# facebookresearch/robust-dynrf

Hardware: AMD Instinct MI355X
Metric: training rays/sec (Nvidia Balloon1, configs/Nvidia.txt, static+dynamic TensorVMSplit) (higher is better)
Workload: dtype f32; 1 GPU; BASELINE.json configs[1]: Nvidia Balloon1, configs/Nvidia.txt, 4096 rays/iter/GPU, 1xMI355X per rank, static+dynamic TensorVMSplit; one step = 5 dynamic + 5 static forward passes, scene-flow MLP, induced flow/disparity, per-frame depth loss, distortion loss, compositor, factor regularisers, full backward, Adam; config=nvidia, stage=stage0, samples_per_ray=115, global_batch=4096, rays_per_gpu=4096, parallelism=ray-sharded dp1, ranks=1, dead_work=executed (work the reference also computes although nothing consumes it)

## Files before the change

include/rodynrf.h:

```cpp
#ifndef RODYNRF_H
#define RODYNRF_H
#include <stddef.h>
#include <stdint.h>

#ifdef __cplusplus
extern "C" {
#endif

#define RDRF_ABI_VERSION 6

typedef void* rdrf_stream_t;

enum { RDRF_RAY_NDC = 0, RDRF_RAY_CONTRACT = 1, RDRF_RAY_OTHER = 2 };
enum { RDRF_ACT_RELU = 0, RDRF_ACT_SOFTPLUS = 1 };
enum { RDRF_HEAD_MLP_FEA = 0, RDRF_HEAD_MLP_FEA_TIMEEMBEDDING = 1 };
enum { RDRF_SCATTER_RAY = 0, RDRF_SCATTER_SORTED = 1, RDRF_SCATTER_AUTO = 2, RDRF_SCATTER_SORTED_PLAIN = 3 };

typedef struct {
  float* plane[3];
  float* line[3];
  int C[3];
  int H[3], W[3];
  int L[3];
  int sH[3], sW[3];
// ... 307 lines not shown
  const uint8_t* masks;
} RdrfSceneTables;
typedef struct RdrfBatch {
  float* rgb;
  float* disp;
  float* fg;
  float* mask_f;
  float* mask_b;
  float* flow_f;
  float* flow_b;
  float* ts;
  float* ts_rand;
  float* grid;
  float* px;
  int64_t* view;
} RdrfBatch;
int rdrf_gather_batch(const RdrfSceneTables* tables, const int64_t* ids, const int64_t* ids2, int N, RdrfBatch* out,
                      rdrf_stream_t stream);

int rdrf_set_scatter_mode(int mode);

int rdrf_deterministic(void);
int rdrf_det_bind(int slot, float* grad_base, size_t n, void* shadow_i64, rdrf_stream_t stream);
int rdrf_det_finish(int slot, rdrf_stream_t stream);

int rdrf_selftest_mlp(const float* x, const float* w, const float* b, int M, int K, int OUT,
                      float* y, void* ws, size_t ws_bytes, rdrf_stream_t stream);

#define RDRF_ST_F32 0
#define RDRF_ST_F32_T 1
#define RDRF_ST_B3 2
#define RDRF_ST_B3_T 3
#define RDRF_ST_B3_PAIR_T 4
#define RDRF_ST_B3S 5
#define RDRF_ST_B3S_T 6
int rdrf_selftest_layer(int form, const float* x, const float* w, int M, int K, int OUT, float* y, void* ws, size_t ws_bytes,
                        rdrf_stream_t stream);

#define RDRF_DW_DENSITY 0
#define RDRF_DW_STATIC_FEA 1
#define RDRF_DW_STATIC_TE 2
#define RDRF_DW_DYN_APP 3
#define RDRF_DW_DYN 4
#define RDRF_DW_SCENE_FLOW 5
#define RDRF_DW_FEAT_STATIC 6
#define RDRF_DW_FEAT_DYN 7
#define RDRF_DW_LIVE_D 1
#define RDRF_DW_LIVE_B 2
#define RDRF_DW_SMALL_IN_KERNEL 4
#define RDRF_DW_WARP_IN_KERNEL 8
int rdrf_selftest_dw(int plan, int flags, const float* A, size_t A_floats, const float* B, size_t B_floats, int ntiles,
                     const int* count, const void* grads, rdrf_stream_t stream);
int rdrf_selftest_dw_describe(int plan, int flags, int* out, int cap);
int rdrf_selftest_sf_geometry(int ntiles, int* grid, int* waves);
int rdrf_selftest_warp_geometry(int ntiles, int* grid, int* waves);
size_t rdrf_selftest_warp_bwd_workspace_bytes(int N, int S);
int rdrf_selftest_warp_bwd(const RdrfDynamicParams* P, const RdrfFieldCfg* cfg, int N, int S, const float* act1,
                           size_t act1_floats, float* grows1, size_t grows1_floats, float* dxw, float* dxn,
                           const float* g_xyz_prime, const RdrfDynamicParams* grads, float* g_xyz, float* dtout, float* dtp,
                           void* ws, size_t ws_bytes, rdrf_stream_t stream);

size_t rdrf_selftest_sort_temp_bytes(unsigned n, int bits);
int rdrf_selftest_sort(const unsigned* keys, unsigned n, int bits, const int* count, unsigned n_mul, unsigned* keys_out,
                       unsigned* order, void* temp, size_t temp_bytes, rdrf_stream_t stream);

#define RDRF_SCK_STATIC_DENSITY 0
#define RDRF_SCK_DYN_DENSITY 1
#define RDRF_SCK_STATIC_APP 2
#define RDRF_SCK_DYN_APP 3
typedef struct {
  RdrfVM vm[2], gvm[2];
  int set_mask;
  int N, S, flat;
  const float* coords;
  float box_lo[3], box_inv[3];
  const unsigned char* valid;
  const int* list;
  const int* count;
  const float* rows;
  size_t rows_floats;
  const float* recs;
  size_t recs_floats;
  float* dxw;
  float* g_xyz;
  void* ws;
  size_t ws_bytes;
  unsigned* keys_out;
  unsigned* keys_sorted_out;
  unsigned* order_out;
  int* counts_out;
} RdrfScatterTest;
size_t rdrf_selftest_scatter_workspace_bytes(int N, int S);
int rdrf_selftest_scatter(int kind, int mode, const RdrfScatterTest* t, rdrf_stream_t stream);
int rdrf_selftest_scatter_describe(int kind, const int* grid, int* out, int cap);
int rdrf_selftest_scatter_last(int* out, int cap);

typedef struct RdrfAlphaMask {
  const uint8_t* bits;
  int grid[3];
  int T;
  float aabb[6];
} RdrfAlphaMask;

size_t rdrf_compute_alpha_workspace_bytes(int M, int T);
int rdrf_compute_alpha(const void* params, int dynamic, const RdrfFieldCfg* cfg, const float* xyz, int M,
                       const float* times, int T, float length, const RdrfAlphaMask* mask, float* alpha, float* sigma,
// ... 19 lines not shown
```

robust-dynrf_amd/_lib.py:

```python
import ctypes as C
import os

import torch

_HERE = os.path.dirname(os.path.abspath(__file__))
DETERMINISTIC = os.environ.get("RDRF_DETERMINISTIC", "0") == "1"
LIB_PATH = os.environ.get("RDRF_LIB", os.path.join(_HERE, "librodynrf_det.so" if DETERMINISTIC else "librodynrf.so"))

ABI_VERSION = 6

RAY_TYPES = {"ndc": 0, "contract": 1}
ACTS = {"relu": 0, "softplus": 1}
HEADS = {"MLP_Fea": 0, "MLP_Fea_TimeEmbedding": 1}
SAVE_NO_APP = 1

fp = C.POINTER(C.c_float)


class RdrfVM(C.Structure):
    _fields_ = [("plane", C.c_void_p * 3), ("line", C.c_void_p * 3), ("C", C.c_int * 3),
                ("H", C.c_int * 3), ("W", C.c_int * 3), ("L", C.c_int * 3),
                ("sH", C.c_int * 3), ("sW", C.c_int * 3)]


# ... 98 lines not shown
                                   C.c_void_p]
    lib.rdrf_pack_floats.restype = C.c_size_t
    lib.rdrf_pack_floats.argtypes = []
    lib.rdrf_loss_terms_workspace_floats.restype = C.c_size_t
    lib.rdrf_loss_terms_workspace_floats.argtypes = [C.c_int]
    lib.rdrf_frame_depth_loss_workspace_bytes.restype = C.c_size_t
    lib.rdrf_frame_depth_loss_workspace_bytes.argtypes = [C.c_int, C.c_int]
    lib.rdrf_frame_depth_loss_fwd.argtypes = [C.c_void_p, C.c_void_p, C.c_void_p, C.c_void_p, C.c_int, C.c_int, C.c_float,
                                              C.c_void_p, C.c_void_p, C.c_void_p, C.c_size_t, C.c_void_p]
    lib.rdrf_frame_depth_loss_bwd.argtypes = [C.c_void_p, C.c_void_p, C.c_void_p, C.c_int, C.c_float, C.c_void_p, C.c_void_p]
    lib.rdrf_render_workspace_bytes.restype = C.c_size_t
    lib.rdrf_render_workspace_bytes.argtypes = [C.c_int, C.c_int]
    lib.rdrf_render_chunks_workspace_bytes.restype = C.c_size_t
    lib.rdrf_render_chunks_workspace_bytes.argtypes = [C.c_int, C.c_int, C.c_int]
    lib.rdrf_render_maps_fwd.argtypes = [C.c_void_p, C.c_void_p, C.c_void_p, C.c_void_p, C.c_void_p, C.c_void_p, C.c_int,
                                         C.c_int, C.c_float, C.c_float, C.c_int, C.POINTER(RenderMapsC), C.c_void_p,
                                         C.c_size_t, C.c_void_p]
    lib.rdrf_render_chunks_maps_fwd.argtypes = [C.c_void_p, C.c_void_p, C.c_void_p, C.c_void_p, C.c_void_p, C.c_void_p,
                                                C.c_int, C.c_int, C.c_int, C.c_float, C.c_float, C.POINTER(RenderMapsC),
                                                C.c_void_p, C.c_size_t, C.c_void_p, C.c_void_p, C.c_int]
    lib.rdrf_render_world_fwd.argtypes = [C.c_void_p, C.c_void_p, C.c_void_p, C.c_void_p, C.c_void_p, C.c_void_p, C.c_int,
                                          C.c_int, C.c_int, C.c_float, C.c_float, C.c_float, C.c_int, C.POINTER(RenderMapsC),
                                          C.c_void_p, C.c_size_t, C.c_void_p, C.c_void_p, C.c_int]
    lib.rdrf_render_motion_workspace_bytes.restype = C.c_size_t
    lib.rdrf_render_motion_workspace_bytes.argtypes = [C.c_int, C.c_int]
    lib.rdrf_render_motion_fwd.argtypes = [C.c_void_p, C.c_void_p, C.c_void_p, C.c_void_p, C.c_void_p, C.c_void_p, C.c_int,
                                           C.c_int, C.c_float, C.c_float, C.c_int, C.POINTER(RenderMapsC),
                                           C.POINTER(MotionCamsC), C.POINTER(MotionMapsC), C.c_void_p, C.c_size_t, C.c_void_p]
    lib.rdrf_flow_to_image_workspace_bytes.restype = C.c_size_t
    lib.rdrf_flow_to_image_workspace_bytes.argtypes = [C.c_int, C.c_int]
    lib.rdrf_flow_to_image.argtypes = [C.c_void_p, C.c_int, C.c_int, C.c_void_p, C.c_void_p, C.c_size_t, C.c_void_p]
    lib.rdrf_camera_rays.argtypes = [C.c_void_p, C.c_void_p, C.c_int, C.c_int, C.c_int, C.c_int, C.c_float, C.c_int64,
                                     C.c_int, C.c_void_p, C.c_void_p]
    lib.rdrf_ssim_workspace_bytes.restype = C.c_size_t
    lib.rdrf_ssim_workspace_bytes.argtypes = [C.c_int, C.c_int, C.c_int]
    lib.rdrf_ssim.argtypes = [C.c_void_p, C.c_void_p, C.c_int, C.c_int, C.c_int, C.c_float, C.c_void_p, C.c_void_p,
                              C.c_void_p, C.c_size_t, C.c_void_p]
    lib.rdrf_compute_alpha_workspace_bytes.restype = C.c_size_t
    lib.rdrf_compute_alpha_workspace_bytes.argtypes = [C.c_int, C.c_int]
    lib.rdrf_compute_alpha.argtypes = [C.c_void_p, C.c_int, C.c_void_p, C.c_void_p, C.c_int, C.c_void_p, C.c_int, C.c_float,
                                       C.POINTER(RdrfAlphaMask), C.c_void_p, C.c_void_p, C.c_void_p, C.c_size_t, C.c_void_p]
    lib.rdrf_alpha_mask_build.argtypes = [C.c_void_p, C.c_int, C.c_int, C.c_int, C.c_int, C.c_float, C.c_void_p, C.c_void_p,
                                          C.c_void_p]
    lib.rdrf_alpha_mask_sample.argtypes = [C.POINTER(RdrfAlphaMask), C.c_void_p, C.c_void_p, C.c_int, C.c_int64, C.c_void_p,
                                           C.c_void_p]
    lib.rdrf_alpha_mask_valid.argtypes = [C.POINTER(RdrfAlphaMask), C.POINTER(RdrfAlphaMask), C.c_void_p, C.c_void_p, C.c_int,
                                          C.c_int, C.c_void_p, C.c_void_p]
    lib.rdrf_gather_batch.argtypes = [C.POINTER(SceneTablesC), C.c_void_p, C.c_void_p, C.c_int, C.POINTER(BatchC), C.c_void_p]
    lib.rdrf_selftest_layer.argtypes = [C.c_int, C.c_void_p, C.c_void_p, C.c_int, C.c_int, C.c_int, C.c_void_p, C.c_void_p,
                                        C.c_size_t, C.c_void_p]
    lib.rdrf_selftest_dw.argtypes = [C.c_int, C.c_int, C.c_void_p, C.c_size_t, C.c_void_p, C.c_size_t, C.c_int, C.c_void_p,
                                     C.c_void_p, C.c_void_p]
    lib.rdrf_selftest_dw_describe.argtypes = [C.c_int, C.c_int, C.POINTER(C.c_int), C.c_int]
    lib.rdrf_selftest_warp_geometry.argtypes = [C.c_int, C.POINTER(C.c_int), C.POINTER(C.c_int)]
    lib.rdrf_selftest_warp_bwd_workspace_bytes.restype = C.c_size_t
    lib.rdrf_selftest_warp_bwd_workspace_bytes.argtypes = [C.c_int, C.c_int]
    lib.rdrf_selftest_warp_bwd.argtypes = [C.c_void_p, C.c_void_p, C.c_int, C.c_int, C.c_void_p, C.c_size_t, C.c_void_p, C.c_size_t,
                                           C.c_void_p, C.c_void_p, C.c_void_p, C.c_void_p, C.c_void_p, C.c_void_p, C.c_void_p,
                                           C.c_void_p, C.c_size_t, C.c_void_p]
    lib.rdrf_selftest_sort_temp_bytes.restype = C.c_size_t
    lib.rdrf_selftest_sort_temp_bytes.argtypes = [C.c_uint, C.c_int]
    lib.rdrf_selftest_sort.argtypes = [C.c_void_p, C.c_uint, C.c_int, C.c_void_p, C.c_uint, C.c_void_p, C.c_void_p, C.c_void_p,
                                       C.c_size_t, C.c_void_p]
    lib.rdrf_selftest_scatter_workspace_bytes.restype = C.c_size_t
    lib.rdrf_selftest_scatter_workspace_bytes.argtypes = [C.c_int, C.c_int]
    lib.rdrf_selftest_scatter.argtypes = [C.c_int, C.c_int, C.POINTER(RdrfScatterTest), C.c_void_p]
    lib.rdrf_selftest_scatter_describe.argtypes = [C.c_int, C.POINTER(C.c_int), C.POINTER(C.c_int), C.c_int]
    lib.rdrf_selftest_scatter_last.argtypes = [C.POINTER(C.c_int), C.c_int]
    lib.rdrf_prof_get.argtypes = [C.c_char_p, C.POINTER(C.c_double), C.POINTER(C.c_int)]
    lib.rdrf_det_bind.argtypes = [C.c_int, C.c_void_p, C.c_size_t, C.c_void_p, C.c_void_p]
    lib.rdrf_det_finish.argtypes = [C.c_int, C.c_void_p]
    if DETERMINISTIC and not lib.rdrf_deterministic():
        raise ImportError(f"RDRF_DETERMINISTIC=1 but {LIB_PATH} is the product build")
    return lib


lib = _load()

SYMBOLS = [
    "rdrf_abi_version", "rdrf_last_error", "rdrf_workspace_bytes", "rdrf_forward_workspace_bytes", "rdrf_saved_bytes", "rdrf_saved_bytes_ex", "rdrf_saved_row_bytes",
    "rdrf_generate_rays",
    "rdrf_generate_rays_bwd", "rdrf_generate_rays_uv", "rdrf_generate_rays_uv_bwd", "rdrf_sample_ndc", "rdrf_sample_contract", "rdrf_sample_bwd",
    "rdrf_sample_world", "rdrf_sample_world_bwd", "rdrf_render_world_fwd",
    "rdrf_static_fwd", "rdrf_static_fwd_ex", "rdrf_static_bwd", "rdrf_dynamic_fwd", "rdrf_dynamic_fwd_ex", "rdrf_dynamic_bwd",
    "rdrf_features_saved_bytes", "rdrf_features_workspace_bytes", "rdrf_features_bwd_workspace_bytes",
    "rdrf_static_features_fwd", "rdrf_static_features_bwd", "rdrf_dynamic_features_fwd",
    "rdrf_dynamic_features_bwd",
    "rdrf_scene_flow_fwd", "rdrf_scene_flow_bwd", "rdrf_composite_fwd", "rdrf_composite_bwd",
    "rdrf_induce_flow_fwd", "rdrf_induce_flow_bwd", "rdrf_rows_scatter_add", "rdrf_distloss_fwd", "rdrf_distloss_bwd",
    "rdrf_tv_fwd", "rdrf_tv_bwd", "rdrf_tv_grad", "rdrf_adam_step", "rdrf_upsample_bilinear", "rdrf_dense_l1_fwd",
    "rdrf_dense_l1_bwd", "rdrf_pack_floats", "rdrf_static_pack", "rdrf_dynamic_pack", "rdrf_loss_terms_workspace_floats", "rdrf_loss_terms_fwd", "rdrf_loss_terms_bwd",
    "rdrf_loss_terms_stats", "rdrf_loss_terms_finish", "rdrf_deterministic", "rdrf_det_bind", "rdrf_det_finish",
    "rdrf_render_fused_fwd", "rdrf_render_sequence_fwd",
    "rdrf_frame_depth_loss_workspace_bytes", "rdrf_frame_depth_loss_fwd", "rdrf_frame_depth_loss_bwd",
    "rdrf_render_workspace_bytes", "rdrf_render_fwd", "rdrf_render_chunks_workspace_bytes", "rdrf_render_chunks_fwd",
    "rdrf_render_maps_fwd", "rdrf_render_chunks_maps_fwd", "rdrf_camera_rays", "rdrf_ssim_workspace_bytes", "rdrf_ssim",
    "rdrf_render_motion_workspace_bytes", "rdrf_render_motion_fwd", "rdrf_flow_to_image_workspace_bytes", "rdrf_flow_to_image",
    "rdrf_gather_batch",
    "rdrf_compute_alpha_workspace_bytes", "rdrf_compute_alpha", "rdrf_alpha_mask_build", "rdrf_alpha_mask_sample",
    "rdrf_alpha_mask_valid",
    "rdrf_set_scatter_mode", "rdrf_selftest_mlp", "rdrf_selftest_layer", "rdrf_selftest_dw", "rdrf_selftest_dw_describe",
    "rdrf_selftest_sf_geometry", "rdrf_selftest_warp_geometry", "rdrf_selftest_warp_bwd_workspace_bytes", "rdrf_selftest_warp_bwd",
    "rdrf_selftest_sort_temp_bytes", "rdrf_selftest_sort", "rdrf_selftest_scatter_workspace_bytes", "rdrf_selftest_scatter",
    "rdrf_selftest_scatter_describe", "rdrf_selftest_scatter_last",
    "rdrf_prof_reset",
    "rdrf_prof_enable", "rdrf_prof_get",
]


SELFTEST_FORMS = {"F32": 0, "F32_T": 1, "B3": 2, "B3_T": 3, "B3_PAIR_T": 4, "B3S": 5, "B3S_T": 6}

DW_PLANS = {"DENSITY": 0, "STATIC_FEA": 1, "STATIC_TE": 2, "DYN_APP": 3, "DYN": 4, "SCENE_FLOW": 5, "FEAT_STATIC": 6, "FEAT_DYN": 7}
DW_LIVE_D, DW_LIVE_B, DW_SMALL_IN_KERNEL, DW_WARP_IN_KERNEL = 1, 2, 4, 8

SCATTER_KINDS = {"STATIC_DENSITY": 0, "DYN_DENSITY": 1, "STATIC_APP": 2, "DYN_APP": 3}

SCATTER_MODES = {"ray": 0, "sorted": 1, "auto": 2, "sorted_plain": 3}


def set_scatter_mode(mode):
    check(lib.rdrf_set_scatter_mode(SCATTER_MODES[mode]), "rdrf_set_scatter_mode")


class RdrfTensor4(C.Structure):
    _fields_ = [("x", C.c_void_p), ("g", C.c_void_p), ("C", C.c_int), ("H", C.c_int), ("W", C.c_int),
                ("sC", C.c_longlong), ("sH", C.c_longlong), ("sW", C.c_longlong)]


TV_MAX = 16


class RdrfLossTerm(C.Structure):
    _fields_ = [("x", C.c_void_p), ("y", C.c_void_p), ("w", C.c_void_p), ("gx", C.c_void_p), ("gy", C.c_void_p),
                ("rows", C.c_longlong), ("cols", C.c_int), ("kind", C.c_int), ("norm", C.c_int),
                ("ysign", C.c_float), ("coef", C.c_float), ("coef_dev", C.c_void_p)]


MAX_LOSS_TERMS = 32


class RdrfError(RuntimeError):
    pass


def check(rc, what):
    if rc != 0:
        raise RdrfError(f"{what} failed (rc={rc}): {lib.rdrf_last_error().decode()}")


def require_device(*tensors):
    for t in tensors:
        if t is not None and not t.is_cuda:
            raise RdrfError("rodynrf ops run on the MI355X only: got a CPU tensor "
                            "(there is no CPU fallback; the oracle lives under oracle/ for tests)")
# ... 50 lines not shown
```

robust-dynrf_amd/csrc/rdrf_bwd_host.hpp:

```cpp
#pragma once
#include "rdrf_host.hpp"

struct BwdArgs;
struct DynG;

struct BwdWs {
  float* dfs;
  float* dfa;
  unsigned *keys_in, *keys_out, *order;
  int* counts;
  void* sort_tmp;
  size_t sort_tmp_bytes;
  float* pk;
  float* gf;
  float* grows1;
  float* grows3;
  float* dxw;
  float* dxn;
  float* dtout;
  float* gsig;
  float* dtp;
};

struct ScatterArgs {
// ... 17 lines not shown
  int bcast;
};
enum ScatterKernel {
  SCATTER_4_1_3,
  SCATTER_4_1_9,
  SCATTER_12_3_9,
  SCATTER_12_3_27
};
void fill_scatter_common(ScatterArgs& sa, const BwdArgs& a);
int launch_scatter(const char* name, ScatterKernel kern, ScatterArgs& sa, long ntiles, hipStream_t stream);
int scatter_mode(size_t ns, hipStream_t stream);
int scatter_dyn_app_sorted(const BwdArgs& a, const BwdWs& b, const RdrfDynamicParams* P, const RdrfDynamicParams* G,
                           hipStream_t stream);
int scatter_dyn_density_sorted(const BwdArgs& a, const BwdWs& b, const RdrfDynamicParams* P, const RdrfDynamicParams* G,
                               int set_mask, hipStream_t stream);
int sorted_key_bits(const int W[3], const int H[3]);
int scatter_mode_swap(int mode);
struct ScatterLaunch {
  int elem_bytes;
  int threads, workgroups;
  int tiled;
  int tw, slice_steps;
};
struct ScatterRecord {
  int form;
  int split;
  int n;
  ScatterLaunch l[4];
};
const ScatterRecord& scatter_last_record();

struct DwJob {
  const float* A;
  int A_stride, A_row0, nbo, out_dim, out_row0;
  const float* B;
  int B_stride;
  int nblk;
  int blk_row0[8], blk_seg[8], blk_e0[8];
  int in_dim, ld;
  float* dW;
  float* db;
  const int* count;
  int ntiles;
};
#define RDRF_MAX_DW_JOBS 12
struct DwJobs {
  DwJob j[RDRF_MAX_DW_JOBS];
  int n;
};
void dw_add(DwJobs& D, const float* A, int A_stride, int A_row0, int nbo, int out_dim, int out_row0, const float* B,
            int B_stride, int in_dim, int ld, float* dW, float* db, const int* count, int ntiles);
void dw_blk(DwJobs& D, int row0, int seg, int e0);
int dw_launch(DwJobs& D, hipStream_t stream, const char* name);

void add_density_phase_dw(DwJobs& D, const float* grows1, const float* act1, const RdrfDynamicParams* G, int T1,
                          bool live_d = true, bool live_b = true, bool small_in_kernel = false, bool warp_in_kernel = false);
void add_static_app_dw(DwJobs& D, const float* grows3, const float* act3, const RdrfStaticParams* G, bool fea, const int* cnt,
                       int ntiles);
void add_dyn_app_dw(DwJobs& D, const float* grows3, const float* act3, const RdrfDynamicParams* G, const int* cnt, int ntiles);
void add_scene_flow_dw(DwJobs& D, const float* grows, const float* act, const RdrfDynamicParams* G, int T);
void add_feat_static_dw(DwJobs& D, const float* grows3, const float* act3, const RdrfStaticParams* G, int Np);
void add_feat_dyn_app_dw(DwJobs& D, const float* grows3, const float* act3, const RdrfDynamicParams* G, int Np);
int warp_bwd_on_rows(const RdrfDynamicParams* P, const RdrfFieldCfg* cfg, int N, int S, const float* act1, float* grows1,
                     float* dxw, float* dxn, const float* g_xyz_prime, const RdrfDynamicParams* G, float* g_xyz, float* dtout,
                     float* dtp, float* pk, uint8_t* valid, hipStream_t stream);
size_t warp_bwd_on_rows_pack_floats();

void fused_dw_geometry(long tiles, int* grid, int* waves);
int launch_scene_flow_fused(int N, int S, const Box& box, const float* pkimg, const float* saved, const float* g_sf_f,
                            const float* g_sf_b, const RdrfDynamicParams* G, float* g_pts, long tiles, hipStream_t stream);
int launch_warp_fused(const BwdArgs& a, const DynG& gw, const RdrfDynamicParams* G, long tiles, hipStream_t stream);
```

robust-dynrf_amd/csrc/rdrf_dw.hip:

```cpp
#include <algorithm>

#include "rdrf_kernels.hpp"
#include "rdrf_bwd_host.hpp"

RDRF_DET_UNIT(dw)

void dw_add(DwJobs& D, const float* A, int A_stride, int A_row0, int nbo, int out_dim,
            int out_row0, const float* B, int B_stride, int in_dim, int ld, float* dW,
            float* db, const int* count, int ntiles) {
  DwJob& j = D.j[D.n];
  memset(&j, 0, sizeof(j));
  j.A = A; j.A_stride = A_stride; j.A_row0 = A_row0; j.nbo = nbo; j.out_dim = out_dim;
  j.out_row0 = out_row0; j.B = B; j.B_stride = B_stride; j.nblk = 0; j.in_dim = in_dim; j.ld = ld;
  j.dW = dW; j.db = db; j.count = count; j.ntiles = ntiles;
  D.n++;
}
void dw_blk(DwJobs& D, int row0, int seg, int e0) {
  DwJob& j = D.j[D.n - 1];
  j.blk_row0[j.nblk] = row0; j.blk_seg[j.nblk] = seg; j.blk_e0[j.nblk] = e0;
  j.nblk++;
}
#define DW2_MAX_BLK 30
#define DW2_MAX_PROD 4
#define DW2_WAVES 12
#define DW2_MAX_SEG 2
struct Dw2Prod {
  int a, b;
  int job, bo, k;
  int bias;
};
struct Dw2Plan {
  const float* A;
  const float* B;
  int A_stride, B_stride;
  int nblk;
  int blk_meta[DW2_MAX_BLK];
  int nseg;
  int seg_blk0[DW2_MAX_SEG];
  int seg_src[DW2_MAX_SEG];
  int seg_row0[DW2_MAX_SEG];
  int nprod[DW2_WAVES];
  Dw2Prod prod[DW2_WAVES][DW2_MAX_PROD];
  const int* count;
  int ntiles;
  DwJob job[RDRF_MAX_DW_JOBS];
};

__global__ __launch_bounds__(64 * DW2_WAVES) void k_dw3(Dw2Plan P) {
  extern __shared__ __attribute__((aligned(16))) f32x4 dw3_stage[];
  const int tid = threadIdx.x, lane = tid & 63, h = lane >> 5, li = lane & 31;
  const int wave = __builtin_amdgcn_readfirstlane(tid >> 6);
  const int ntiles = P.count ? ((*P.count + 31) >> 5) : P.ntiles;
  static_assert(DW2_MAX_SEG == 2 && (DW2_WAVES & 1) == 0, "segment select below; a wave's pieces share their parity");
  const int sb1 = P.nseg > 1 ? P.seg_blk0[1] : 1 << 20;
  const int s1 = P.nseg > 1 ? 1 : 0;
  const float* seg0a = (P.seg_src[0] ? P.B : P.A) + (size_t)P.seg_row0[0] * 32;
  const float* seg0b = (P.seg_src[s1] ? P.B : P.A) + (size_t)P.seg_row0[s1] * 32 - (size_t)P.seg_blk0[s1] * 1024;
  const size_t st0 = (size_t)(P.seg_src[0] ? P.B_stride : P.A_stride) * 32,
               st1 = (size_t)(P.seg_src[s1] ? P.B_stride : P.A_stride) * 32;
  const int npieces = 2 * P.nblk;
  constexpr int NPW = (2 * DW2_MAX_BLK + DW2_WAVES - 1) / DW2_WAVES;
  const int prow_ = 16 * (wave & 1) + (lane >> 2);
  const unsigned voff = (unsigned)(prow_ * 128 + (((lane & 3) ^ ((prow_ >> 2) & 3)) << 4));
  const int hbuf = P.nblk * 128;
  auto dma = [&](int t, int hf, int buf) {
    const float* g0 = seg0a + (size_t)t * st0;
    const float* g1 = seg0b + (size_t)t * st1;
    const __amdgpu_buffer_rsrc_t r0 = __builtin_amdgcn_make_buffer_rsrc((void*)g0, 0, 0x7fffffff, 0x00020000);
    const __amdgpu_buffer_rsrc_t r1 = __builtin_amdgcn_make_buffer_rsrc((void*)g1, 0, 0x7fffffff, 0x00020000);
#pragma unroll
    for (int i = 0; i < NPW; ++i) {
      const int pc = wave + DW2_WAVES * i;
      if (pc < npieces) {
        const int blk = pc >> 1;
        __attribute__((address_space(3))) void* dst = (__attribute__((address_space(3))) void*)(dw3_stage + buf * hbuf + pc * 64);
        const unsigned soff = (unsigned)(blk * 4096 + hf * 64);
        if (blk < sb1) __builtin_amdgcn_raw_ptr_buffer_load_lds(r0, dst, 16, voff, soff, 0, 0);
        else __builtin_amdgcn_raw_ptr_buffer_load_lds(r1, dst, 16, voff, soff, 0, 0);
      }
    }
  };
  int rpos[2];
#pragma unroll
  for (int q = 0; q < 2; ++q) rpos[q] = li * 4 + ((2 * h + q) ^ ((li >> 2) & 3));
  const int np = P.nprod[wave];
  int pa[DW2_MAX_PROD], pb[DW2_MAX_PROD];
#pragma unroll
  for (int p = 0; p < DW2_MAX_PROD; ++p) {
    pa[p] = __builtin_amdgcn_readfirstlane(P.prod[wave][p].a * 128 | (P.prod[wave][p].bias << 30));
    pb[p] = __builtin_amdgcn_readfirstlane(P.prod[wave][p].b * 128);
  }
  f32x16 acc[DW2_MAX_PROD];
  float bsum[DW2_MAX_PROD];
#pragma unroll
  for (int p = 0; p < DW2_MAX_PROD; ++p) {
    bsum[p] = 0.f;
#pragma unroll
    for (int r = 0; r < 16; ++r) acc[p][r] = 0.f;
  }
  int t = blockIdx.x, hf = 0, buf = 0;
  if (t < ntiles) dma(t, 0, 0);
  while (t < ntiles) {
    __builtin_amdgcn_s_waitcnt(0x0f70);
    __syncthreads();
    int tn = t, hn = hf ^ 1;
    if (hf) tn = t + gridDim.x;
    if (tn < ntiles) dma(tn, hn, buf ^ 1);
    __builtin_amdgcn_sched_barrier(0);
    const f32x4* stage = dw3_stage + buf * hbuf;
#pragma unroll
    for (int p = 0; p < DW2_MAX_PROD; ++p) {
      if (p < np) {
        int oa = pa[p] & 0xffffff, ob = pb[p];
        asm volatile("" : "+s"(oa), "+s"(ob));
        const f32x4* sa = stage + oa;
        const f32x4* sb = stage + ob;
        f32x4 av4[2], bv4[2];
#pragma unroll
        for (int q = 0; q < 2; ++q) { av4[q] = sa[rpos[q]]; bv4[q] = sb[rpos[q]]; }
        if (pa[p] >> 30) {
#pragma unroll
          for (int q = 0; q < 2; ++q) bsum[p] += av4[q].x + av4[q].y + av4[q].z + av4[q].w;
        }
#pragma unroll
        for (int q = 0; q < 2; ++q) {
          acc[p] = __builtin_amdgcn_mfma_f32_32x32x2f32(av4[q].x, bv4[q].x, acc[p], 0, 0, 0);
          acc[p] = __builtin_amdgcn_mfma_f32_32x32x2f32(av4[q].y, bv4[q].y, acc[p], 0, 0, 0);
          acc[p] = __builtin_amdgcn_mfma_f32_32x32x2f32(av4[q].z, bv4[q].z, acc[p], 0, 0, 0);
          acc[p] = __builtin_amdgcn_mfma_f32_32x32x2f32(av4[q].w, bv4[q].w, acc[p], 0, 0, 0);
        }
      }
    }
    t = tn; hf = hn; buf ^= 1;
  }
#pragma unroll
  for (int p = 0; p < DW2_MAX_PROD; ++p) {
    if (p < np) {
      const Dw2Prod pr = P.prod[wave][p];
      const DwJob& J = P.job[pr.job];
      const int col = seg_imap(J.blk_seg[pr.k], J.blk_e0[pr.k] + li, J.in_dim);
#pragma unroll
      for (int rr = 0; rr < 16; ++rr) {
        const int orow = pr.bo * 32 + (rr & 3) + 8 * (rr >> 2) + 4 * h - J.out_row0;
        if (col >= 0 && orow >= 0 && orow < J.out_dim) grad_add(J.dW + (size_t)orow * J.ld + col, acc[p][rr]);
      }
      if (pr.bias && J.db != nullptr) {
        const float b = bsum[p] + __shfl_xor(bsum[p], 32, 64);
        const int orow = pr.bo * 32 + li - J.out_row0;
        if (h == 0 && orow >= 0 && orow < J.out_dim) grad_add(J.db + orow, b);
      }
    }
  }
}

int dw_launch(DwJobs& D, hipStream_t stream, const char* name) {
  bool done[RDRF_MAX_DW_JOBS] = {false};
  for (int g0 = 0; g0 < D.n; ++g0) {
    if (done[g0]) continue;
    const DwJob& R = D.j[g0];
    Dw2Plan P;
    auto reset = [&]() {
      memset(&P, 0, sizeof(P));
      P.A = R.A; P.B = R.B; P.A_stride = R.A_stride; P.B_stride = R.B_stride;
      P.count = R.count; P.ntiles = R.ntiles;
      for (int i = 0; i < D.n; ++i) P.job[i] = D.j[i];
    };
    auto find_blk = [&](int src, int row) {
      for (int i = 0; i < P.nblk; ++i)
        if (P.blk_meta[i] == ((src << 16) | row)) return i;
      return -1;
    };
    auto flush = [&]() -> int {
      int tot = 0;
      for (int w = 0; w < DW2_WAVES; ++w) tot += P.nprod[w];
      if (tot == 0) return 0;
      {
        for (int src = 0; src < 2; ++src) {
          int lo = 1 << 30, hi = -1;
          for (int i = 0; i < P.nblk; ++i)
            if ((P.blk_meta[i] >> 16) == src) { const int r = P.blk_meta[i] & 0xffff; lo = r < lo ? r : lo; hi = r > hi ? r : hi; }
          for (int r = lo; r < hi; r += 32)
            if (find_blk(src, r) < 0) {
              RDRF_CHECK(P.nblk < DW2_MAX_BLK, -2, "dw: %d staged blocks are not enough to bridge the row ranges of this plan", DW2_MAX_BLK);
              P.blk_meta[P.nblk++] = (src << 16) | r;
            }
        }
      }
      {
        int order[DW2_MAX_BLK], rank[DW2_MAX_BLK], meta[DW2_MAX_BLK];
        for (int i = 0; i < P.nblk; ++i) order[i] = i;
        std::sort(order, order + P.nblk, [&](int x, int y) { return P.blk_meta[x] < P.blk_meta[y]; });
        for (int i = 0; i < P.nblk; ++i) { rank[order[i]] = i; meta[i] = P.blk_meta[order[i]]; }
        for (int i = 0; i < P.nblk; ++i) P.blk_meta[i] = meta[i];
        for (int w = 0; w < DW2_WAVES; ++w)
          for (int k = 0; k < P.nprod[w]; ++k) { P.prod[w][k].a = rank[P.prod[w][k].a]; P.prod[w][k].b = rank[P.prod[w][k].b]; }
        P.nseg = 0;
        for (int i = 0; i < P.nblk; ++i) {
          if (i == 0 || (meta[i] >> 16) != (meta[i - 1] >> 16) || (meta[i] & 0xffff) != (meta[i - 1] & 0xffff) + 32) {
            RDRF_CHECK(P.nseg < DW2_MAX_SEG, -2, "dw: the staged rows form more than %d contiguous runs", DW2_MAX_SEG);
            P.seg_blk0[P.nseg] = i; P.seg_src[P.nseg] = meta[i] >> 16; P.seg_row0[P.nseg] = meta[i] & 0xffff;
            ++P.nseg;
          }
        }
      }
      const size_t lds = (size_t)P.nblk * 4096;
      int grid = 256;
      if (P.count == nullptr && P.ntiles < grid) grid = P.ntiles < 1 ? 1 : P.ntiles;
      if (lds > 48 * 1024)
        RDRF_HIP(hipFuncSetAttribute((const void*)k_dw3, hipFuncAttributeMaxDynamicSharedMemorySize, DW2_MAX_BLK * 4096));
      rdrf_prof_begin(name, stream);
      hipLaunchKernelGGL(k_dw3, dim3(grid), dim3(64 * DW2_WAVES), lds, stream, P);
      rdrf_prof_end(name, stream);
      RDRF_HIP(hipGetLastError());
      return 0;
    };
    reset();
    int nprods = 0;
    for (int ji = g0; ji < D.n; ++ji) {
      const DwJob& J = D.j[ji];
      if (done[ji] || J.A != R.A || J.B != R.B || J.A_stride != R.A_stride || J.B_stride != R.B_stride ||
          J.count != R.count || J.ntiles != R.ntiles)
        continue;
      done[ji] = true;
      for (int bo = 0; bo < J.nbo; ++bo)
        for (int k = 0; k < J.nblk; ++k) {
          int need = (find_blk(0, J.A_row0 + 32 * bo) < 0) + (find_blk(1, J.blk_row0[k]) < 0);
          if (nprods == DW2_WAVES * DW2_MAX_PROD || P.nblk + need > DW2_MAX_BLK) {
            int rc = flush();
            if (rc) return rc;
            reset();
            nprods = 0;
          }
          int a = find_blk(0, J.A_row0 + 32 * bo);
          if (a < 0) { a = P.nblk++; P.blk_meta[a] = J.A_row0 + 32 * bo; }
          int b = find_blk(1, J.blk_row0[k]);
          if (b < 0) { b = P.nblk++; P.blk_meta[b] = (1 << 16) | J.blk_row0[k]; }
          const int w = nprods % DW2_WAVES;
          Dw2Prod& pr = P.prod[w][P.nprod[w]++];
          pr.a = a; pr.b = b; pr.job = ji; pr.bo = bo; pr.k = k;
          pr.bias = (k == 0 && J.db != nullptr) ? 1 : 0;
          ++nprods;
        }
    }
    int rc = flush();
    if (rc) return rc;
  }
  return 0;
}
```

robust-dynrf_amd/csrc/rdrf_selftest.hip:

```cpp
#include <vector>

#include "rdrf_bwd_dev.hpp"
#include "rdrf_bwd_host.hpp"

namespace {

template <int KK>
RDRF_D void st_load(float (&in)[KK], const float* __restrict__ x, int row, int M, int ld, int c0, int h) {
#pragma unroll
  for (int kk = 0; kk < KK; ++kk) in[kk] = row < M ? x[(size_t)row * ld + c0 + elem_of(kk, h)] : 0.f;
}
template <int NBO>
RDRF_D void st_store(const f32x16 (&acc)[NBO], float* __restrict__ y, int row, int M, int ld, int c0, int h) {
  if (row < M)
#pragma unroll
    for (int nb = 0; nb < NBO; ++nb)
#pragma unroll
      for (int r = 0; r < 16; ++r) y[(size_t)row * ld + c0 + nb * 32 + elem_of(r, h)] = acc[nb][r];
}

template <int NBO, int KK>
__global__ __launch_bounds__(64) void k_st_f32(const float* __restrict__ x, const float* __restrict__ pkw, int M,
                                               float* __restrict__ y) {
  constexpr int IMG = NBO * KK * 64;
// ... 245 lines not shown
  int rc = dw_plan_jobs(plan, flags, A, B, (size_t)ntiles, count, grads, D, I);
  if (rc) return rc;
  size_t needA = 0, needB = 0;
  for (int g = 0, j = 0; g < I.nregions; ++g) {
    while (j < D.n && I.region[j] != g) ++j;
    needA += (size_t)ntiles * D.j[j].A_stride * 32;
    needB += (size_t)ntiles * D.j[j].B_stride * 32;
  }
  RDRF_CHECK(A_floats >= needA && B_floats >= needB, -3, "selftest_dw: rows too small (A %zu < %zu or B %zu < %zu floats)", A_floats,
             needA, B_floats, needB);
  bool uses_count = false;
  for (int j = 0; j < D.n; ++j) uses_count |= D.j[j].count != nullptr;
  if (uses_count) {
    int c = -1;
    RDRF_HIP(hipMemcpyAsync(&c, count, sizeof(int), hipMemcpyDeviceToHost, stream));
    RDRF_HIP(hipStreamSynchronize(stream));
    RDRF_CHECK(c >= 0 && ((size_t)c + 31) / 32 <= (size_t)ntiles, -1, "selftest_dw: count %d does not fit %d tiles", c, ntiles);
  }
  return dw_launch(D, stream, "selftest_dw");
}

extern "C" int rdrf_selftest_dw_describe(int plan, int flags, int* out, int cap) {
  constexpr size_t NSLOT = (sizeof(RdrfDynamicParams) > sizeof(RdrfStaticParams) ? sizeof(RdrfDynamicParams) : sizeof(RdrfStaticParams)) / 8;
  uintptr_t slots[NSLOT];
  for (size_t i = 0; i < NSLOT; ++i) slots[i] = (i + 1) * 8;
  alignas(16) static const float rowsA[4] = {0.f}, rowsB[4] = {0.f};
  static const int cnt = 0;
  DwJobs D;
  DwPlanInfo I;
  int rc = dw_plan_jobs(plan, flags, rowsA, rowsB, 1, &cnt, slots, D, I);
  if (rc) return rc;
  int need = 4 + 3 * I.nregions;
  for (int j = 0; j < D.n; ++j) need += 10 + 33 * D.j[j].nblk;
  RDRF_CHECK(out != nullptr && cap >= need, -3, "selftest_dw_describe: description buffer too small (%d < %d ints)", out ? cap : 0, need);
  int n = 0;
  out[n++] = need; out[n++] = I.nregions; out[n++] = D.n; out[n++] = I.dynamic;
  for (int g = 0, j = 0; g < I.nregions; ++g) {
    while (j < D.n && I.region[j] != g) ++j;
    out[n++] = D.j[j].A_stride; out[n++] = D.j[j].B_stride; out[n++] = D.j[j].count != nullptr ? 1 : 0;
  }
  for (int j = 0; j < D.n; ++j) {
    const DwJob& J = D.j[j];
    out[n++] = I.region[j]; out[n++] = J.A_row0; out[n++] = J.nbo; out[n++] = J.out_dim; out[n++] = J.out_row0;
    out[n++] = J.in_dim; out[n++] = J.ld;
    out[n++] = (int)((uintptr_t)J.dW - 8);
    out[n++] = J.db != nullptr ? (int)((uintptr_t)J.db - 8) : -1;
    out[n++] = J.nblk;
    for (int k = 0; k < J.nblk; ++k) {
      out[n++] = J.blk_row0[k];
      for (int li = 0; li < 32; ++li) out[n++] = seg_imap(J.blk_seg[k], J.blk_e0[k] + li, J.in_dim);
    }
  }
  return n;
}

extern "C" int rdrf_selftest_sf_geometry(int ntiles, int* grid, int* waves) {
  RDRF_CHECK(ntiles >= 0 && grid && waves, -1, "selftest_sf_geometry: bad arguments");
  fused_dw_geometry(ntiles, grid, waves);
  return 0;
}

extern "C" int rdrf_selftest_warp_geometry(int ntiles, int* grid, int* waves) {
  RDRF_CHECK(ntiles >= 0 && grid && waves, -1, "selftest_warp_geometry: bad arguments");
  fused_dw_geometry(ntiles, grid, waves);
  return 0;
}

extern "C" size_t rdrf_selftest_warp_bwd_workspace_bytes(int N, int S) {
  return warp_bwd_on_rows_pack_floats() * 4 + (((size_t)N * S + 255) & ~(size_t)255) + 512;
}
extern "C" int rdrf_selftest_warp_bwd(const RdrfDynamicParams* P, const RdrfFieldCfg* cfg, int N, int S, const float* act1,
                                      size_t act1_floats, float* grows1, size_t grows1_floats, float* dxw, float* dxn,
                                      const float* g_xyz_prime, const RdrfDynamicParams* grads, float* g_xyz, float* dtout,
                                      float* dtp, void* ws, size_t ws_bytes, rdrf_stream_t stream_) {
  hipStream_t stream = (hipStream_t)stream_;
  if (N == 0) return 0;
  RDRF_CHECK(P && cfg && grads && act1 && grows1 && dxw && dxn && dtout && dtp && ws && N > 0 && S > 0 && S <= 4096, -1,
             "selftest_warp_bwd: bad arguments");
  RDRF_CHECK((size_t)N * S * 3 < (size_t)INT32_MAX, -1, "selftest_warp_bwd: N * S * 3 must stay below 2^31");
  RDRF_CHECK((((uintptr_t)act1 | (uintptr_t)grows1 | (uintptr_t)ws) & 15) == 0, -1, "selftest_warp_bwd: rows and workspace must be 16-byte aligned");
  const size_t tiles = ((size_t)N * S + 31) / 32;
  RDRF_CHECK(act1_floats >= tiles * sv::K1_ROWS * 32 && grows1_floats >= tiles * sv::K1G_ROWS * 32, -3,
             "selftest_warp_bwd: rows too small for %zu tiles", tiles);
  RDRF_CHECK(ws_bytes >= rdrf_selftest_warp_bwd_workspace_bytes(N, S), -3, "selftest_warp_bwd: workspace too small");
  WsCarver c(ws, ws_bytes);
  float* pk = c.take<float>(warp_bwd_on_rows_pack_floats());
  uint8_t* valid = c.take<uint8_t>((size_t)N * S);
  return warp_bwd_on_rows(P, cfg, N, S, act1, grows1, dxw, dxn, g_xyz_prime, grads, g_xyz, dtout, dtp, pk, valid, stream);
}

extern "C" size_t rdrf_selftest_sort_temp_bytes(unsigned n, int bits) { return rdrf_sort_temp_bytes(n, bits); }

extern "C" int rdrf_selftest_sort(const unsigned* keys, unsigned n, int bits, const int* count, unsigned n_mul, unsigned* keys_out,
                                  unsigned* order, void* temp, size_t temp_bytes, rdrf_stream_t stream_) {
  hipStream_t stream = (hipStream_t)stream_;
  RDRF_CHECK(bits >= 1 && bits <= 32, -1, "selftest_sort: bits must be 1 .. 32 (got %d)", bits);
  if (n == 0) return 0;
  RDRF_CHECK(keys && keys_out && order, -1, "selftest_sort: bad arguments (null keys, keys_out or order)");
  RDRF_CHECK(count == nullptr || n_mul >= 1, -1, "selftest_sort: a device count needs n_mul >= 1");
  RDRF_CHECK(temp != nullptr && (((uintptr_t)temp) & 255) == 0, -1, "selftest_sort: the temporary storage must be 256-byte aligned");
  if (count) {
    int c = -1;
    RDRF_HIP(hipMemcpyAsync(&c, count, sizeof(int), hipMemcpyDeviceToHost, stream));
    RDRF_HIP(hipStreamSynchronize(stream));
    RDRF_CHECK(c >= 0 && (unsigned long long)c * n_mul <= 0xffffffffull, -1, "selftest_sort: device count %d out of range", c);
  }
// ... 212 lines not shown
```

Baseline: 468,800 rays/s.

## Template dW kernel on accumulator count and bridge only small gaps between row runs

The weight-gradient kernel k_dw3 is now templated on the number of accumulators per wave. Plans where no wave holds more than two products use a 2-accumulator variant with fewer registers, launched with up to two workgroups per CU when LDS allows. Segment handling grows from two to four contiguous runs, with per-piece base pointers computed once. Row-range bridging now fills only the smallest gaps until at most four runs remain, instead of filling every gap per source, which cuts staged blocks and DMA traffic. It also adds a plan-description selftest, at the cost of two kernel instantiations and more host planning logic.

```diff
diff --git a/include/rodynrf.h b/include/rodynrf.h
--- a/include/rodynrf.h
+++ b/include/rodynrf.h
@@ -383,6 +383,7 @@
 int rdrf_selftest_dw(int plan, int flags, const float* A, size_t A_floats, const float* B, size_t B_floats, int ntiles,
                      const int* count, const void* grads, rdrf_stream_t stream);
 int rdrf_selftest_dw_describe(int plan, int flags, int* out, int cap);
+int rdrf_selftest_dw_plan(int plan, int flags, int ntiles, int* out, int cap);
 int rdrf_selftest_sf_geometry(int ntiles, int* grid, int* waves);
 int rdrf_selftest_warp_geometry(int ntiles, int* grid, int* waves);
 size_t rdrf_selftest_warp_bwd_workspace_bytes(int N, int S);
diff --git a/robust-dynrf_amd/_lib.py b/robust-dynrf_amd/_lib.py
--- a/robust-dynrf_amd/_lib.py
+++ b/robust-dynrf_amd/_lib.py
@@ -174,6 +174,7 @@
     lib.rdrf_selftest_dw.argtypes = [C.c_int, C.c_int, C.c_void_p, C.c_size_t, C.c_void_p, C.c_size_t, C.c_int, C.c_void_p,
                                      C.c_void_p, C.c_void_p]
     lib.rdrf_selftest_dw_describe.argtypes = [C.c_int, C.c_int, C.POINTER(C.c_int), C.c_int]
+    lib.rdrf_selftest_dw_plan.argtypes = [C.c_int, C.c_int, C.c_int, C.POINTER(C.c_int), C.c_int]
     lib.rdrf_selftest_warp_geometry.argtypes = [C.c_int, C.POINTER(C.c_int), C.POINTER(C.c_int)]
     lib.rdrf_selftest_warp_bwd_workspace_bytes.restype = C.c_size_t
     lib.rdrf_selftest_warp_bwd_workspace_bytes.argtypes = [C.c_int, C.c_int]
@@ -222,6 +223,7 @@
     "rdrf_compute_alpha_workspace_bytes", "rdrf_compute_alpha", "rdrf_alpha_mask_build", "rdrf_alpha_mask_sample",
     "rdrf_alpha_mask_valid",
     "rdrf_set_scatter_mode", "rdrf_selftest_mlp", "rdrf_selftest_layer", "rdrf_selftest_dw", "rdrf_selftest_dw_describe",
+    "rdrf_selftest_dw_plan",
     "rdrf_selftest_sf_geometry", "rdrf_selftest_warp_geometry", "rdrf_selftest_warp_bwd_workspace_bytes", "rdrf_selftest_warp_bwd",
     "rdrf_selftest_sort_temp_bytes", "rdrf_selftest_sort", "rdrf_selftest_scatter_workspace_bytes", "rdrf_selftest_scatter",
     "rdrf_selftest_scatter_describe", "rdrf_selftest_scatter_last",
diff --git a/robust-dynrf_amd/csrc/rdrf_bwd_host.hpp b/robust-dynrf_amd/csrc/rdrf_bwd_host.hpp
--- a/robust-dynrf_amd/csrc/rdrf_bwd_host.hpp
+++ b/robust-dynrf_amd/csrc/rdrf_bwd_host.hpp
@@ -93,6 +93,7 @@
             int B_stride, int in_dim, int ld, float* dW, float* db, const int* count, int ntiles);
 void dw_blk(DwJobs& D, int row0, int seg, int e0);
 int dw_launch(DwJobs& D, hipStream_t stream, const char* name);
+int dw_describe_launches(const DwJobs& D, int* out, int cap);
 
 void add_density_phase_dw(DwJobs& D, const float* grows1, const float* act1, const RdrfDynamicParams* G, int T1,
                           bool live_d = true, bool live_b = true, bool small_in_kernel = false, bool warp_in_kernel = false);
diff --git a/robust-dynrf_amd/csrc/rdrf_dw.hip b/robust-dynrf_amd/csrc/rdrf_dw.hip
--- a/robust-dynrf_amd/csrc/rdrf_dw.hip
+++ b/robust-dynrf_amd/csrc/rdrf_dw.hip
@@ -1,4 +1,5 @@
 #include <algorithm>
+#include <vector>
 
 #include "rdrf_kernels.hpp"
 #include "rdrf_bwd_host.hpp"
@@ -23,7 +24,7 @@
 #define DW2_MAX_BLK 30
 #define DW2_MAX_PROD 4
 #define DW2_WAVES 12
-#define DW2_MAX_SEG 2
+#define DW2_MAX_SEG 4
 struct Dw2Prod {
   int a, b;
   int job, bo, k;
@@ -46,37 +47,43 @@
   DwJob job[RDRF_MAX_DW_JOBS];
 };
 
+template <int NACC>
 __global__ __launch_bounds__(64 * DW2_WAVES) void k_dw3(Dw2Plan P) {
   extern __shared__ __attribute__((aligned(16))) f32x4 dw3_stage[];
   const int tid = threadIdx.x, lane = tid & 63, h = lane >> 5, li = lane & 31;
   const int wave = __builtin_amdgcn_readfirstlane(tid >> 6);
   const int ntiles = P.count ? ((*P.count + 31) >> 5) : P.ntiles;
-  static_assert(DW2_MAX_SEG == 2 && (DW2_WAVES & 1) == 0, "segment select below; a wave's pieces share their parity");
-  const int sb1 = P.nseg > 1 ? P.seg_blk0[1] : 1 << 20;
-  const int s1 = P.nseg > 1 ? 1 : 0;
-  const float* seg0a = (P.seg_src[0] ? P.B : P.A) + (size_t)P.seg_row0[0] * 32;
-  const float* seg0b = (P.seg_src[s1] ? P.B : P.A) + (size_t)P.seg_row0[s1] * 32 - (size_t)P.seg_blk0[s1] * 1024;
-  const size_t st0 = (size_t)(P.seg_src[0] ? P.B_stride : P.A_stride) * 32,
-               st1 = (size_t)(P.seg_src[s1] ? P.B_stride : P.A_stride) * 32;
+  static_assert((DW2_WAVES & 1) == 0, "a wave's pieces share their parity");
   const int npieces = 2 * P.nblk;
   constexpr int NPW = (2 * DW2_MAX_BLK + DW2_WAVES - 1) / DW2_WAVES;
+  const float* pbase[NPW];
+  unsigned pstep[NPW];
+#pragma unroll
+  for (int i = 0; i < NPW; ++i) {
+    const int blk = (wave + DW2_WAVES * i) >> 1;
+    int src = P.seg_src[0], row0 = P.seg_row0[0], b0 = 0;
+#pragma unroll
+    for (int q = 1; q < DW2_MAX_SEG; ++q) {
+      const bool in = blk >= P.seg_blk0[q];
+      src = in ? P.seg_src[q] : src; row0 = in ? P.seg_row0[q] : row0; b0 = in ? P.seg_blk0[q] : b0;
+    }
+    pbase[i] = (src ? P.B : P.A) + (ptrdiff_t)row0 * 32 - (ptrdiff_t)b0 * 1024;
+    pstep[i] = (unsigned)(src ? P.B_stride : P.A_stride) * 32u;
+  }
   const int prow_ = 16 * (wave & 1) + (lane >> 2);
   const unsigned voff = (unsigned)(prow_ * 128 + (((lane & 3) ^ ((prow_ >> 2) & 3)) << 4));
   const int hbuf = P.nblk * 128;
   auto dma = [&](int t, int hf, int buf) {
-    const float* g0 = seg0a + (size_t)t * st0;
-    const float* g1 = seg0b + (size_t)t * st1;
-    const __amdgpu_buffer_rsrc_t r0 = __builtin_amdgcn_make_buffer_rsrc((void*)g0, 0, 0x7fffffff, 0x00020000);
-    const __amdgpu_buffer_rsrc_t r1 = __builtin_amdgcn_make_buffer_rsrc((void*)g1, 0, 0x7fffffff, 0x00020000);
 #pragma unroll
     for (int i = 0; i < NPW; ++i) {
       const int pc = wave + DW2_WAVES * i;
       if (pc < npieces) {
         const int blk = pc >> 1;
+        const float* g = pbase[i] + (size_t)t * pstep[i];
+        const __amdgpu_buffer_rsrc_t r = __builtin_amdgcn_make_buffer_rsrc((void*)g, 0, 0x7fffffff, 0x00020000);
         __attribute__((address_space(3))) void* dst = (__attribute__((address_space(3))) void*)(dw3_stage + buf * hbuf + pc * 64);
         const unsigned soff = (unsigned)(blk * 4096 + hf * 64);
-        if (blk < sb1) __builtin_amdgcn_raw_ptr_buffer_load_lds(r0, dst, 16, voff, soff, 0, 0);
-        else __builtin_amdgcn_raw_ptr_buffer_load_lds(r1, dst, 16, voff, soff, 0, 0);
+        __builtin_amdgcn_raw_ptr_buffer_load_lds(r, dst, 16, voff, soff, 0, 0);
       }
     }
   };
@@ -84,16 +91,16 @@
 #pragma unroll
   for (int q = 0; q < 2; ++q) rpos[q] = li * 4 + ((2 * h + q) ^ ((li >> 2) & 3));
   const int np = P.nprod[wave];
-  int pa[DW2_MAX_PROD], pb[DW2_MAX_PROD];
-#pragma unroll
-  for (int p = 0; p < DW2_MAX_PROD; ++p) {
+  int pa[NACC], pb[NACC];
+#pragma unroll
+  for (int p = 0; p < NACC; ++p) {
     pa[p] = __builtin_amdgcn_readfirstlane(P.prod[wave][p].a * 128 | (P.prod[wave][p].bias << 30));
     pb[p] = __builtin_amdgcn_readfirstlane(P.prod[wave][p].b * 128);
   }
-  f32x16 acc[DW2_MAX_PROD];
-  float bsum[DW2_MAX_PROD];
-#pragma unroll
-  for (int p = 0; p < DW2_MAX_PROD; ++p) {
+  f32x16 acc[NACC];
+  float bsum[NACC];
+#pragma unroll
+  for (int p = 0; p < NACC; ++p) {
     bsum[p] = 0.f;
 #pragma unroll
     for (int r = 0; r < 16; ++r) acc[p][r] = 0.f;
@@ -109,7 +116,7 @@
     __builtin_amdgcn_sched_barrier(0);
     const f32x4* stage = dw3_stage + buf * hbuf;
 #pragma unroll
-    for (int p = 0; p < DW2_MAX_PROD; ++p) {
+    for (int p = 0; p < NACC; ++p) {
       if (p < np) {
         int oa = pa[p] & 0xffffff, ob = pb[p];
         asm volatile("" : "+s"(oa), "+s"(ob));
@@ -134,7 +141,7 @@
     t = tn; hf = hn; buf ^= 1;
   }
 #pragma unroll
-  for (int p = 0; p < DW2_MAX_PROD; ++p) {
+  for (int p = 0; p < NACC; ++p) {
     if (p < np) {
       const Dw2Prod pr = P.prod[wave][p];
       const DwJob& J = P.job[pr.job];
@@ -153,7 +160,70 @@
   }
 }
 
-int dw_launch(DwJobs& D, hipStream_t stream, const char* name) {
+struct DwLaunch {
+  Dw2Plan P;
+  int grid, lds;
+  int nacc;
+};
+#define DW2_LDS_PER_CU (160 * 1024)
+#define DW2_WG_PER_CU_2ACC 2
+
+static int dw_close_plan(Dw2Plan& P, std::vector<DwLaunch>& out) {
+  int tot = 0, most = 0;
+  for (int w = 0; w < DW2_WAVES; ++w) { tot += P.nprod[w]; most = P.nprod[w] > most ? P.nprod[w] : most; }
+  if (tot == 0) return 0;
+  auto count_runs = [&](const int* meta, int n) {
+    int runs = 0;
+    for (int i = 0; i < n; ++i) runs += i == 0 || meta[i] != meta[i - 1] + 32;
+    return runs;
+  };
+  for (;;) {
+    int meta[DW2_MAX_BLK];
+    for (int i = 0; i < P.nblk; ++i) meta[i] = P.blk_meta[i];
+    std::sort(meta, meta + P.nblk);
+    if (count_runs(meta, P.nblk) <= DW2_MAX_SEG) break;
+    int best = -1, best_n = 1 << 30;
+    for (int i = 1; i < P.nblk; ++i) {
+      if ((meta[i] >> 16) != (meta[i - 1] >> 16)) continue;
+      const int n = ((meta[i] & 0xffff) - (meta[i - 1] & 0xffff)) / 32 - 1;
+      if (n > 0 && n < best_n) { best = i; best_n = n; }
+    }
+    RDRF_CHECK(best >= 0 && P.nblk + best_n <= DW2_MAX_BLK, -2,
+               "dw: the staged rows form more than %d contiguous runs and %d staged blocks are not enough to bridge them", DW2_MAX_SEG,
+               DW2_MAX_BLK);
+    for (int r = (meta[best - 1] & 0xffff) + 32; r < (meta[best] & 0xffff); r += 32) P.blk_meta[P.nblk++] = (meta[best] & ~0xffff) | r;
+  }
+  {
+    int order[DW2_MAX_BLK], rank[DW2_MAX_BLK], meta[DW2_MAX_BLK];
+    for (int i = 0; i < P.nblk; ++i) order[i] = i;
+    std::sort(order, order + P.nblk, [&](int x, int y) { return P.blk_meta[x] < P.blk_meta[y]; });
+    for (int i = 0; i < P.nblk; ++i) { rank[order[i]] = i; meta[i] = P.blk_meta[order[i]]; }
+    for (int i = 0; i < P.nblk; ++i) P.blk_meta[i] = meta[i];
+    for (int w = 0; w < DW2_WAVES; ++w)
+      for (int k = 0; k < P.nprod[w]; ++k) { P.prod[w][k].a = rank[P.prod[w][k].a]; P.prod[w][k].b = rank[P.prod[w][k].b]; }
+    P.nseg = 0;
+    for (int i = 0; i < P.nblk; ++i) {
+      if (i == 0 || meta[i] != meta[i - 1] + 32) {
+        RDRF_CHECK(P.nseg < DW2_MAX_SEG, -2, "dw: the staged rows form more than %d contiguous runs", DW2_MAX_SEG);
+        P.seg_blk0[P.nseg] = i; P.seg_src[P.nseg] = meta[i] >> 16; P.seg_row0[P.nseg] = meta[i] & 0xffff;
+        ++P.nseg;
+      }
+    }
+    for (int q = P.nseg; q < DW2_MAX_SEG; ++q) P.seg_blk0[q] = 1 << 20;
+  }
+  DwLaunch L;
+  L.lds = P.nblk * 4096;
+  L.nacc = most <= 2 ? 2 : DW2_MAX_PROD;
+  int per_cu = DW2_LDS_PER_CU / L.lds;
+  if (per_cu > (L.nacc == 2 ? DW2_WG_PER_CU_2ACC : 1)) per_cu = L.nacc == 2 ? DW2_WG_PER_CU_2ACC : 1;
+  L.grid = 256 * per_cu;
+  if (P.count == nullptr && P.ntiles < L.grid) L.grid = P.ntiles < 1 ? 1 : P.ntiles;
+  L.P = P;
+  out.push_back(L);
+  return 0;
+}
+
+static int dw_plan(const DwJobs& D, std::vector<DwLaunch>& out) {
   bool done[RDRF_MAX_DW_JOBS] = {false};
   for (int g0 = 0; g0 < D.n; ++g0) {
     if (done[g0]) continue;
@@ -170,50 +240,6 @@
         if (P.blk_meta[i] == ((src << 16) | row)) return i;
       return -1;
     };
-    auto flush = [&]() -> int {
-      int tot = 0;
-      for (int w = 0; w < DW2_WAVES; ++w) tot += P.nprod[w];
-      if (tot == 0) return 0;
-      {
-        for (int src = 0; src < 2; ++src) {
-          int lo = 1 << 30, hi = -1;
-          for (int i = 0; i < P.nblk; ++i)
-            if ((P.blk_meta[i] >> 16) == src) { const int r = P.blk_meta[i] & 0xffff; lo = r < lo ? r : lo; hi = r > hi ? r : hi; }
-          for (int r = lo; r < hi; r += 32)
-            if (find_blk(src, r) < 0) {
-              RDRF_CHECK(P.nblk < DW2_MAX_BLK, -2, "dw: %d staged blocks are not enough to bridge the row ranges of this plan", DW2_MAX_BLK);
-              P.blk_meta[P.nblk++] = (src << 16) | r;
-            }
-        }
-      }
-      {
-        int order[DW2_MAX_BLK], rank[DW2_MAX_BLK], meta[DW2_MAX_BLK];
-        for (int i = 0; i < P.nblk; ++i) order[i] = i;
-        std::sort(order, order + P.nblk, [&](int x, int y) { return P.blk_meta[x] < P.blk_meta[y]; });
-        for (int i = 0; i < P.nblk; ++i) { rank[order[i]] = i; meta[i] = P.blk_meta[order[i]]; }
-        for (int i = 0; i < P.nblk; ++i) P.blk_meta[i] = meta[i];
-        for (int w = 0; w < DW2_WAVES; ++w)
-          for (int k = 0; k < P.nprod[w]; ++k) { P.prod[w][k].a = rank[P.prod[w][k].a]; P.prod[w][k].b = rank[P.prod[w][k].b]; }
-        P.nseg = 0;
-        for (int i = 0; i < P.nblk; ++i) {
-          if (i == 0 || (meta[i] >> 16) != (meta[i - 1] >> 16) || (meta[i] & 0xffff) != (meta[i - 1] & 0xffff) + 32) {
-            RDRF_CHECK(P.nseg < DW2_MAX_SEG, -2, "dw: the staged rows form more than %d contiguous runs", DW2_MAX_SEG);
-            P.seg_blk0[P.nseg] = i; P.seg_src[P.nseg] = meta[i] >> 16; P.seg_row0[P.nseg] = meta[i] & 0xffff;
-            ++P.nseg;
-          }
-        }
-      }
-      const size_t lds = (size_t)P.nblk * 4096;
-      int grid = 256;
-      if (P.count == nullptr && P.ntiles < grid) grid = P.ntiles < 1 ? 1 : P.ntiles;
-      if (lds > 48 * 1024)
-        RDRF_HIP(hipFuncSetAttribute((const void*)k_dw3, hipFuncAttributeMaxDynamicSharedMemorySize, DW2_MAX_BLK * 4096));
-      rdrf_prof_begin(name, stream);
-      hipLaunchKernelGGL(k_dw3, dim3(grid), dim3(64 * DW2_WAVES), lds, stream, P);
-      rdrf_prof_end(name, stream);
-      RDRF_HIP(hipGetLastError());
-      return 0;
-    };
     reset();
     int nprods = 0;
     for (int ji = g0; ji < D.n; ++ji) {
@@ -226,7 +252,7 @@
         for (int k = 0; k < J.nblk; ++k) {
           int need = (find_blk(0, J.A_row0 + 32 * bo) < 0) + (find_blk(1, J.blk_row0[k]) < 0);
           if (nprods == DW2_WAVES * DW2_MAX_PROD || P.nblk + need > DW2_MAX_BLK) {
-            int rc = flush();
+            int rc = dw_close_plan(P, out);
             if (rc) return rc;
             reset();
             nprods = 0;
@@ -242,8 +268,58 @@
           ++nprods;
         }
     }
-    int rc = flush();
+    int rc = dw_close_plan(P, out);
     if (rc) return rc;
   }
   return 0;
 }
+
+int dw_describe_launches(const DwJobs& D, int* out, int cap) {
+  std::vector<DwLaunch> Ls;
+  int rc = dw_plan(D, Ls);
+  if (rc) return rc;
+  int need = 2;
+  for (const DwLaunch& L : Ls) {
+    need += 5 + 3 * L.P.nseg + 2 * L.P.nblk + DW2_WAVES;
+    for (int w = 0; w < DW2_WAVES; ++w) need += 5 * L.P.nprod[w];
+  }
+  RDRF_CHECK(out != nullptr && cap >= need, -3, "selftest_dw_plan: description buffer too small (%d < %d ints)", out ? cap : 0, need);
+  int n = 0;
+  out[n++] = need; out[n++] = (int)Ls.size();
+  for (const DwLaunch& L : Ls) {
+    const Dw2Plan& P = L.P;
+    out[n++] = L.grid; out[n++] = L.lds; out[n++] = L.nacc; out[n++] = P.nblk; out[n++] = P.nseg;
+    for (int q = 0; q < P.nseg; ++q) { out[n++] = P.seg_src[q]; out[n++] = P.seg_row0[q]; out[n++] = P.seg_blk0[q]; }
+    for (int i = 0; i < P.nblk; ++i) { out[n++] = P.blk_meta[i] >> 16; out[n++] = P.blk_meta[i] & 0xffff; }
+    for (int w = 0; w < DW2_WAVES; ++w) {
+      out[n++] = P.nprod[w];
+      for (int k = 0; k < P.nprod[w]; ++k) {
+        const Dw2Prod& pr = P.prod[w][k];
+        out[n++] = pr.a; out[n++] = pr.b; out[n++] = pr.job; out[n++] = pr.bo; out[n++] = pr.k;
+      }
+    }
+  }
+  return n;
+}
+
+template <int NACC>
+static int dw_launch_one(const DwLaunch& L, hipStream_t stream, const char* name) {
+  if (L.lds > 48 * 1024)
+    RDRF_HIP(hipFuncSetAttribute((const void*)k_dw3<NACC>, hipFuncAttributeMaxDynamicSharedMemorySize, DW2_MAX_BLK * 4096));
+  rdrf_prof_begin(name, stream);
+  hipLaunchKernelGGL(k_dw3<NACC>, dim3(L.grid), dim3(64 * DW2_WAVES), (size_t)L.lds, stream, L.P);
+  rdrf_prof_end(name, stream);
+  RDRF_HIP(hipGetLastError());
+  return 0;
+}
+
+int dw_launch(DwJobs& D, hipStream_t stream, const char* name) {
+  std::vector<DwLaunch> Ls;
+  int rc = dw_plan(D, Ls);
+  if (rc) return rc;
+  for (const DwLaunch& L : Ls) {
+    rc = L.nacc == 2 ? dw_launch_one<2>(L, stream, name) : dw_launch_one<DW2_MAX_PROD>(L, stream, name);
+    if (rc) return rc;
+  }
+  return 0;
+}
diff --git a/robust-dynrf_amd/csrc/rdrf_selftest.hip b/robust-dynrf_amd/csrc/rdrf_selftest.hip
--- a/robust-dynrf_amd/csrc/rdrf_selftest.hip
+++ b/robust-dynrf_amd/csrc/rdrf_selftest.hip
@@ -321,6 +321,22 @@
     }
   }
   return n;
+}
+
+extern "C" int rdrf_selftest_dw_plan(int plan, int flags, int ntiles, int* out, int cap) {
+  constexpr size_t NSLOT = (sizeof(RdrfDynamicParams) > sizeof(RdrfStaticParams) ? sizeof(RdrfDynamicParams) : sizeof(RdrfStaticParams)) / 8;
+  uintptr_t slots[NSLOT];
+  for (size_t i = 0; i < NSLOT; ++i) slots[i] = (i + 1) * 8;
+  alignas(16) static const float rowsA[4] = {0.f}, rowsB[4] = {0.f};
+  static const int cnt = 0;
+  RDRF_CHECK(ntiles >= 1 && ntiles <= (1 << 20), -1, "selftest_dw_plan: bad arguments (ntiles = %d)", ntiles);
+  DwJobs D;
+  DwPlanInfo I;
+  int rc = dw_plan_jobs(plan, flags, rowsA, rowsB, 0, &cnt, slots, D, I);
+  if (rc) return rc;
+  for (int j = 0; j < D.n; ++j)
+    if (D.j[j].count == nullptr) D.j[j].ntiles = ntiles;
+  return dw_describe_launches(D, out, cap);
 }
 
 extern "C" int rdrf_selftest_sf_geometry(int ntiles, int* grid, int* waves) {
```

New measurement: 480,400 rays/s (median of 6 runs). +2.5%, better.
